# WU-CVGL/SIU3R

Hardware: AMD Instinct MI355X
Metric: image-pairs/sec @2x512^2 (SIU3R network forward incl. panoptic post-process) (higher is better)
Workload: dtype bf16x3 (fp32 activations, bf16 MFMA with hi/lo operand split; meets the 1e-3 parity bar)

## Files before the change

include/siu3r_hip.h:

```cpp
#ifndef SIU3R_HIP_H
#define SIU3R_HIP_H
#include <stdint.h>
#ifdef __cplusplus
extern "C" {
#endif

#define SIU3R_BF16 0
#define SIU3R_F32 1
#define SIU3R_F16 2
#define SIU3R_F64 3

const char* siu3r_last_error(void);
#define SIU3R_ABI_VERSION 12
int siu3r_abi_version(void);

int siu3r_rope2d(void* tokens, int dtype, int B, int N, int H, int D, int64_t stride_b,
                 int64_t stride_n, int64_t stride_h, const int64_t* positions, float base, float fwd,
                 void* stream);

typedef struct {
  const void* a;
  const void* w_hi;
  const void* w_lo;
  void* c;
// ... 62 lines not shown
int siu3r_layernorm2(const float* x, void* y, int y_dtype, void* y2_bf16, const float* gamma, const float* beta, int64_t rows, int C,
                     int64_t ldx, int64_t ldy, int64_t ldy2, float eps, void* stream);

typedef struct {
  const void *q, *k, *v;
  void* out;
  int32_t dtype;
  int32_t B, H, Nq, Nk, D;
  int64_t q_sb, q_sn, q_sh, k_sb, k_sn, k_sh, v_sb, v_sn, v_sh;
  float scale;
  const float *rope_cos, *rope_sin;
  int32_t rope_max_pos;
  const int64_t *qpos, *kpos;
  const uint8_t* mask;
  int32_t split3;
  int64_t mask_ld;
  float* ws;
  int32_t splits;
  int32_t kv_bxor;
  int32_t kv_x3;
  int32_t out_x3;
} siu3r_attn_params;
int siu3r_attention(const siu3r_attn_params* p, void* stream);
int siu3r_attention_out_x3_ok(const siu3r_attn_params* p);
int siu3r_attention_kv_x3_ok(const siu3r_attn_params* p);
typedef struct {
  char kernel[160];
  int32_t queries_per_wg, key_ranges, combine, key_halves, side_path;
} siu3r_attn_plan_t;
int siu3r_attention_plan(const siu3r_attn_params* p, siu3r_attn_plan_t* out);

int siu3r_add(const float* a, const float* b, float* y, int64_t rows, int64_t b_rows, int C, void* stream);
int siu3r_pack_image_nhwc(const float* img, void* out, int out_dtype, int N, int H, int W, int cpad, void* stream);
int siu3r_resize_bilinear(const void* x, int x_dtype, void* y, int y_dtype, const void* addend, int add_dtype,
                          const float* ch_scale, const float* ch_shift, int N, int IH, int IW, int OH, int OW,
                          int C, int align_corners, void* stream);
int siu3r_resize_bilinear_strided(const void* x, int x_dtype, void* y, int y_dtype, const void* addend, int add_dtype,
                                  const float* ch_scale, const float* ch_shift, int N, int IH, int IW, int OH, int OW,
                                  int C, int align_corners, int64_t x_batch_stride, int64_t addend_batch_stride, void* stream);
int siu3r_resize_bilinear_planes(const void* x, int x_dtype, void* y_planes, int N, int IH, int IW, int OH, int OW, int C, int align_corners,
                                 int64_t x_batch_stride, void* stream);
int siu3r_affine_add(const void* x, int x_dtype, const void* addend, int add_dtype, void* y, int y_dtype,
                     const float* ch_scale, const float* ch_shift, int64_t rows, int C, void* stream);
int siu3r_affine_add_strided(const void* x, int x_dtype, const void* addend, int add_dtype, void* y, int y_dtype,
                             const float* ch_scale, const float* ch_shift, int64_t rows, int C, int64_t rows_per_batch,
                             int64_t x_batch_stride, int64_t addend_batch_stride, void* stream);
int siu3r_maxpool3x3s2(const void* x, void* y, int dtype, int N, int IH, int IW, int C, void* stream);
int siu3r_maxpool2x2s2(const void* x, void* y, int dtype, int N, int IH, int IW, int C, void* stream);
int siu3r_lpips_layer(const float* f0, const float* f1, const float* w, float* dist, int64_t npix, int C, float eps, void* stream);
int siu3r_stem7x7_x3(const float* img, const void* wfrag, const float* bias, const float* up_src, float* out, int B, int G, int H, int W,
                     int planes_out, void* stream);
int siu3r_proj_rows_x3(const float* x, const void* wfrag, const float* bias, float* out, int Z, int G, int64_t M, int K, int N, int ldc,
                       int64_t out_z_stride, void* stream);
int siu3r_dwconv3x3_gelu(const void* x, void* y, int dtype, const float* w9c, const float* bias, int B, int H,
                         int W, int C, void* stream);
int siu3r_dwconv3x3_gelu_planes(const float* x, void* y_planes, const float* w9c, const float* bias, int B, int H, int W, int C, void* stream);
int siu3r_msdeform_sample(const void* value, int v_dtype, const float* offs_aw, const float* ref,
                          const int32_t* shapes_host, void* out, int out_dtype, int B, int S, int Q, int heads,
                          int d, int L, int P, void* stream);
int siu3r_msdeform_sample_planes(const void* value, int v_dtype, const float* offs_aw, const float* ref, const int32_t* shapes_host,
                                 void* out_planes, int B, int S, int Q, int heads, int d, int L, int P, void* stream);
int siu3r_groupnorm(const void* x, int x_dtype, void* y, int y_dtype, const float* gamma, const float* beta,
                    float* stats_ws, const void* addend, int add_dtype, int relu, int N, int HW, int C,
                    int groups, float eps, void* stream);
int siu3r_pts3d_exp(float* xyz, int64_t n, void* stream);
int siu3r_gaussian_adapter(const void* raw, int raw_dtype, float* opacities, float* scales, float* rotations,
                           float* harmonics, float* covariances, int64_t n, void* stream);
int siu3r_m2f_attn_mask(const float* mask_logits, uint8_t* out, int32_t* row_counts_ws, int B, int T, int IH,
                        int IW, int OH, int OW, int Q, int64_t out_ld, void* stream);

typedef struct {
  int32_t mode;
  int32_t width, height;
  float w2c[16];
  float proj[16];
  float tanfovx, tanfovy;
  float campos[3];
  float bg[3];
  int32_t sh_degree;
  int32_t sh_band4;
  float k2_znear_cull;
  float fx, fy, cx, cy;
  float near_plane, far_plane;
  float eps2d;
  float radius_clip;
  float extent_sigma;
  int32_t opacity_aware_extent;
  float alpha_min;
  float alpha_max;
  float t_min;
  float dilation;
  int32_t nt_post_blend;
  float k2_near, k2_far;
} siu3r_raster_cam;
int siu3r_raster_geometry(int width, int height, int64_t G, int32_t* out8);
int siu3r_raster_project(const siu3r_raster_cam* cams_host, int V, void* cams_dev, int64_t G, const float* means, const float* cov,
                         int cov_stride, const float* opacities, const float* colors, int channels, int sh_planar, float* rec,
                         int32_t* radii, int32_t* rect, int32_t* tiles_touched, uint32_t* keys, uint64_t* stats, void* stream);
int siu3r_raster_project_dp(const siu3r_raster_cam* cams_host, int V, void* cams_dev, const float* viewmats_dev, const float* Ks_dev, int64_t G,
                            const float* means, const float* cov, int cov_stride, const float* opacities, const float* colors, int channels,
                            int sh_planar, float* rec, int32_t* radii, int32_t* rect, int32_t* tiles_touched, uint32_t* keys, uint64_t* stats,
                            void* stream);
int siu3r_raster_project_c2w(const siu3r_raster_cam* cams_host, int V, void* cams_dev, const float* c2w_dev, const float* Kn_dev, float t_scale,
                             int64_t G, const float* means, const float* cov, int cov_stride, const float* opacities, const float* colors,
                             int channels, int sh_planar, float* rec, int32_t* radii, int32_t* rect, int32_t* tiles_touched, uint32_t* keys,
                             uint64_t* stats, void* stream);
// ... 158 lines not shown
```

siu3r_amd/_lib.py:

```python
from __future__ import annotations

import ctypes as C
import os

_HERE = os.path.dirname(os.path.abspath(__file__))
LIB_PATH = os.environ.get("SIU3R_LIB_OVERRIDE") or os.path.join(_HERE, "libsiu3r_hip.so")

BF16, F32 = 0, 1


class GemmParams(C.Structure):
    _fields_ = [
        ("a", C.c_void_p), ("w_hi", C.c_void_p), ("w_lo", C.c_void_p), ("c", C.c_void_p),
        ("bias", C.c_void_p), ("residual", C.c_void_p),
        ("m", C.c_int32), ("n", C.c_int32), ("k", C.c_int32), ("kpad", C.c_int32),
        ("lda", C.c_int64), ("ldc", C.c_int64), ("ldr", C.c_int64),
        ("a_dtype", C.c_int32), ("c_dtype", C.c_int32), ("r_dtype", C.c_int32),
        ("act", C.c_int32), ("relu_in", C.c_int32),
        ("batch", C.c_int32),
        ("sa", C.c_int64), ("sw", C.c_int64), ("sc", C.c_int64), ("sr", C.c_int64),
        ("a_mode", C.c_int32),
        ("ih", C.c_int32), ("iw", C.c_int32), ("cin", C.c_int32), ("kh", C.c_int32), ("kw", C.c_int32),
        ("stride", C.c_int32), ("pad", C.c_int32), ("oh", C.c_int32), ("ow", C.c_int32),
        ("out_mode", C.c_int32), ("up", C.c_int32), ("cout", C.c_int32),
# ... 41 lines not shown
        ("key_halves", C.c_int32), ("side_path", C.c_int32),
    ]


class RasterCam(C.Structure):
    _fields_ = [
        ("mode", C.c_int32), ("width", C.c_int32), ("height", C.c_int32),
        ("w2c", C.c_float * 16), ("proj", C.c_float * 16),
        ("tanfovx", C.c_float), ("tanfovy", C.c_float), ("campos", C.c_float * 3), ("bg", C.c_float * 3),
        ("sh_degree", C.c_int32), ("sh_band4", C.c_int32), ("k2_znear_cull", C.c_float),
        ("fx", C.c_float), ("fy", C.c_float), ("cx", C.c_float), ("cy", C.c_float),
        ("near_plane", C.c_float), ("far_plane", C.c_float), ("eps2d", C.c_float), ("radius_clip", C.c_float),
        ("extent_sigma", C.c_float), ("opacity_aware_extent", C.c_int32),
        ("alpha_min", C.c_float), ("alpha_max", C.c_float), ("t_min", C.c_float), ("dilation", C.c_float),
        ("nt_post_blend", C.c_int32), ("k2_near", C.c_float), ("k2_far", C.c_float),
    ]


class AdamField(C.Structure):
    _fields_ = [
        ("param", C.c_void_p), ("grad", C.c_void_p), ("exp_avg", C.c_void_p), ("exp_avg_sq", C.c_void_p),
        ("width", C.c_int32), ("head_period", C.c_int32), ("lr", C.c_float), ("lr_tail", C.c_float),
    ]


_P, _I, _L, _F = C.c_void_p, C.c_int, C.c_int64, C.c_float
ABI_VERSION = 12

SIGNATURES = {
    "siu3r_last_error": [],
    "siu3r_abi_version": [],
    "siu3r_rope2d": [_P, _I, _I, _I, _I, _I, _L, _L, _L, _P, _F, _F, _P],
    "siu3r_gemm": [C.POINTER(GemmParams), _P],
    "siu3r_gemm_plan": [C.POINTER(GemmParams), C.POINTER(GemmPlan)],
    "siu3r_gemm_tune": [_I, _I],
    "siu3r_layernorm": [_P, _P, _I, _P, _P, _L, _I, _L, _L, _F, _P],
    "siu3r_layernorm2": [_P, _P, _I, _P, _P, _P, _L, _I, _L, _L, _L, _F, _P],
    "siu3r_attention": [C.POINTER(AttnParams), _P],
    "siu3r_attention_kv_x3_ok": [C.POINTER(AttnParams)],
    "siu3r_attention_out_x3_ok": [C.POINTER(AttnParams)],
    "siu3r_attention_plan": [C.POINTER(AttnParams), C.POINTER(AttnPlan)],
    "siu3r_add": [_P, _P, _P, _L, _L, _I, _P],
    "siu3r_pack_image_nhwc": [_P, _P, _I, _I, _I, _I, _I, _P],
    "siu3r_resize_bilinear": [_P, _I, _P, _I, _P, _I, _P, _P, _I, _I, _I, _I, _I, _I, _I, _P],
    "siu3r_affine_add": [_P, _I, _P, _I, _P, _I, _P, _P, _L, _I, _P],
    "siu3r_resize_bilinear_strided": [_P, _I, _P, _I, _P, _I, _P, _P, _I, _I, _I, _I, _I, _I, _I, _L, _L, _P],
    "siu3r_resize_bilinear_planes": [_P, _I, _P, _I, _I, _I, _I, _I, _I, _I, _L, _P],
    "siu3r_affine_add_strided": [_P, _I, _P, _I, _P, _I, _P, _P, _L, _I, _L, _L, _L, _P],
    "siu3r_maxpool3x3s2": [_P, _P, _I, _I, _I, _I, _I, _P],
    "siu3r_maxpool2x2s2": [_P, _P, _I, _I, _I, _I, _I, _P],
    "siu3r_lpips_layer": [_P, _P, _P, _P, _L, _I, _F, _P],
    "siu3r_stem7x7_x3": [_P, _P, _P, _P, _P, _I, _I, _I, _I, _I, _P],
    "siu3r_proj_rows_x3": [_P, _P, _P, _P, _I, _I, _L, _I, _I, _I, _L, _P],
    "siu3r_dwconv3x3_gelu": [_P, _P, _I, _P, _P, _I, _I, _I, _I, _P],
    "siu3r_dwconv3x3_gelu_planes": [_P, _P, _P, _P, _I, _I, _I, _I, _P],
    "siu3r_msdeform_sample_planes": [_P, _I, _P, _P, C.POINTER(C.c_int32), _P, _I, _I, _I, _I, _I, _I, _I, _P],
    "siu3r_msdeform_sample": [_P, _I, _P, _P, C.POINTER(C.c_int32), _P, _I, _I, _I, _I, _I, _I, _I, _I, _P],
    "siu3r_groupnorm": [_P, _I, _P, _I, _P, _P, _P, _P, _I, _I, _I, _I, _I, _I, _F, _P],
    "siu3r_pts3d_exp": [_P, _L, _P],
    "siu3r_gaussian_adapter": [_P, _I, _P, _P, _P, _P, _P, _L, _P],
    "siu3r_m2f_attn_mask": [_P, _P, _P, _I, _I, _I, _I, _I, _I, _I, _L, _P],
    "siu3r_split_bf16": [_P, _P, _P, _P, _L, _I, _I, _L, _P],
    "siu3r_raster_geometry": [_I, _I, _L, C.POINTER(C.c_int32)],
    "siu3r_raster_project": [C.POINTER(RasterCam), _I, _P, _L, _P, _P, _I, _P, _P, _I, _I, _P, _P, _P, _P, _P, _P, _P],
    "siu3r_raster_sort": [_I, _L, _P, _P, _P, _P, _P, _P, _P, _P],
    "siu3r_raster_bin": [C.POINTER(RasterCam), _I, _L, _P, _P, _P, _P, _P, _P, _P, _L, _P, _P],
    "siu3r_raster_composite_rgb": [C.POINTER(RasterCam), _I, _P, _L, _P, _P, _L, _P, _P, _P, _P, _P, _P],
    "siu3r_raster_tile_lists": [C.POINTER(RasterCam), _I, _P, _P, _L, _P, _P, _P, _L, _P, _P],
    "siu3r_raster_composite_feat": [C.POINTER(RasterCam), _I, _P, _L, _P, _P, _L, _P, _P, _I, _P, _P, _P],
    "siu3r_raster_composite_feat_ws_bytes": [_I, _I, _I, _L],
    "siu3r_raster_tune": [_I, _I],
    "siu3r_raster_composite_feat_ws": [C.POINTER(RasterCam), _I, _P, _L, _P, _P, _L, _P, _P, _I, _P, _P, _P, _L, _P],
    "siu3r_scale_inplace": [_P, _L, _F, _P],
    "siu3r_quat_scale_to_cov6": [_P, _P, _P, _L, _P],
    "siu3r_sh_eval": [_P, _P, _P, _I, _I, _P, _L, _P],
    "siu3r_blend_background": [_P, _P, _P, _I, _L, _P],
    "siu3r_sh_eval_dp": [_P, _P, _P, _I, _I, _P, _L, _P],
    "siu3r_blend_background_dp": [_P, _P, _P, _I, _L, _P],
    "siu3r_raster_project_dp": [C.POINTER(RasterCam), _I, _P, _P, _P, _L, _P, _P, _I, _P, _P, _I, _I, _P, _P, _P, _P, _P, _P, _P],
    "siu3r_raster_project_c2w": [C.POINTER(RasterCam), _I, _P, _P, _P, _F, _L, _P, _P, _I, _P, _P, _I, _I, _P, _P, _P, _P, _P, _P, _P],
    "siu3r_raster_project_aa": [C.POINTER(RasterCam), _I, _P, _L, _P, _P, _I, _P, _P, _I, _I, _P, _P, _P, _P, _P, _P, _P, _P],
    "siu3r_raster_project_c2w_aa": [C.POINTER(RasterCam), _I, _P, _P, _P, _F, _L, _P, _P, _I, _P, _P, _I, _I, _P, _P, _P, _P, _P, _P, _P, _P],
    "siu3r_raster_project_bwd_aa": [C.POINTER(RasterCam), _I, _P, _L, _P, _P, _I, _P, _P, _I, _I, _P, _P, _P, _P, _P, _P, _P, _P, _P],
    "siu3r_mip_filter3d_ws": [_I],
    "siu3r_mip_filter3d": [_P, _P, _I, _I, _I, _P, _L, _F, _F, _F, _P, _P, _P],
    "siu3r_mip_apply": [_P, _P, _P, _L, _P, _P, _P],
    "siu3r_mip_apply_bwd": [_P, _P, _P, _P, _P, _L, _P, _P, _P],
    "siu3r_raster_composite_rgb_bwd": [C.POINTER(RasterCam), _I, _P, _L, _P, _P, _L, _P, _P, _P, _P, _P, _P, _P, _P, _P],
    "siu3r_raster_composite_rgb_bwd_abs": [C.POINTER(RasterCam), _I, _P, _L, _P, _P, _L, _P, _P, _P, _P, _P, _P, _P, _P, _P, _P],
    "siu3r_raster_contrib": [C.POINTER(RasterCam), _I, _P, _L, _P, _P, _L, _P, _P, _P, _P, _P],
    "siu3r_raster_project_bwd": [C.POINTER(RasterCam), _I, _P, _L, _P, _P, _I, _P, _P, _I, _I, _P, _P, _P, _P, _P, _P, _P, _P, _P],
    "siu3r_raster_pose_partial_rows": [_L],
    "siu3r_raster_pose_reduce": [_I, _L, _P, _P, _P],
    "siu3r_raster_composite_rgb_bwd_k3": [C.POINTER(RasterCam), _I, _P, _L, _P, _P, _L, _P, _P, _P, _P, _P, _P, _P],
    "siu3r_raster_composite_feat_ws_lists": [_I, _I, _I, _L, _P, _I, _P, _L, _L],
    "siu3r_raster_quad_lists": [C.POINTER(RasterCam), _I, _P, _L, _P, _P, _L, _P, _P, _L, _P],
    "siu3r_raster_composite_feat_bwd": [C.POINTER(RasterCam), _I, _P, _L, _P, _P, _L, _P, _P, _I, _P, _P, _P, _P, _P, _P, _P],
    "siu3r_raster_project_bwd_k3": [C.POINTER(RasterCam), _I, _P, _L, _P, _P, _I, _P, _P, _P, _P, _P, _P, _P, _P],
    "siu3r_raster_viewmat_reduce": [_I, _L, _P, _P, _P],
    "siu3r_quat_scale_to_cov6_bwd": [_P, _P, _P, _P, _P, _L, _P],
    "siu3r_sh_eval_bwd": [_P, _P, _P, _I, _I, _P, _P, _P, _P, _L, _P],
    "siu3r_photo_loss_partials": [_I, _I, _I, _I],
    "siu3r_photo_loss": [_P, _P, _I, _I, _I, _I, C.POINTER(C.c_int64), C.POINTER(C.c_int64), _F, _F, _P, _P, _P, _P],
    "siu3r_depth_loss_ws": [_I, _I, _I],
    "siu3r_depth_loss": [_P, _P, _P, _P, _I, _I, _I, _I, _I, _F, _P, _P, _P, _P, _P, _P, _P],
    "siu3r_depth_smooth_ws": [_I, _I, _I],
# ... 68 lines not shown
```

siu3r_amd/model.py:

```python
from __future__ import annotations

import functools
import math
from typing import Dict, List, Optional, Sequence

import os

import torch
import torch.nn.functional as F

from . import ops
from .ops import ACT_GELU, ACT_NONE, ACT_RELU
from .gaussians_types import Gaussians
from . import postprocess as pp

ENC_HEADS, DEC_HEADS = 16, 12
ADAPTER_IDX = (5, 11, 17, 23)
DPT_HOOKS = (0, 6, 9, 12)


class _Weights:

    def __init__(self, sd: Dict[str, torch.Tensor], device, split: bool):
        self.sd, self.dev, self.split = sd, device, split
# ... 5 lines not shown

    def v(self, name):
        if name not in self.vec:
            self.vec[name] = self.t(name).contiguous()
        return self.vec[name]

    def linear(self, name, key=None, extra_bias=None):
        key = key or name
        if key not in self.lin:
            w = self.t(name + ".weight")
            w = w.reshape(w.shape[0], -1)
            b = self.t(name + ".bias") if (name + ".bias") in self.sd else None
            if extra_bias is not None:
                b = extra_bias if b is None else b + extra_bias
            self.lin[key] = ops.pack_matrix(w, b, self.split)
        return self.lin[key]

    def linear_ln(self, names, ln_name, eps=1e-6):
        names = [names] if isinstance(names, str) else list(names)
        key = "+".join(names) + "#ln:" + ln_name
        if key not in self.lin:
            w = torch.cat([self.t(n + ".weight").reshape(self.sd[n + ".weight"].shape[0], -1) for n in names], 0)
            b = torch.cat([self.t(n + ".bias") for n in names], 0) if (names[0] + ".bias") in self.sd else None
            pw = ops.pack_linear_ln(w, b, self.t(ln_name + ".weight"), self.t(ln_name + ".bias"), self.split)
            pw.meta["ln_eps"] = eps
            self.lin[key] = pw
        return self.lin[key]

    def linear_ln_rows(self, name, rows, ln_name, eps=1e-6):
        key = f"{name}[{rows[0]}:{rows[1]}]#ln:{ln_name}"
        if key not in self.lin:
            w = self.t(name + ".weight")[rows[0]:rows[1]]
            b = self.t(name + ".bias")[rows[0]:rows[1]] if (name + ".bias") in self.sd else None
            pw = ops.pack_linear_ln(w, b, self.t(ln_name + ".weight"), self.t(ln_name + ".bias"), self.split)
            pw.meta["ln_eps"] = eps
            self.lin[key] = pw
        return self.lin[key]

    def group(self, key, build, prefixes):
        if key not in self.lin:
            self.lin[key] = ops.stack_packed([build(q) for q in prefixes])
        return self.lin[key]

    def stem7(self, names):
        key = "stem7:" + "|".join(names)
        if key not in self.lin:
            self.lin[key] = ops.pack_stem7([self.t(n + ".weight") for n in names], [self.t(n + ".bias") if (n + ".bias") in self.sd else None for n in names])
        return self.lin[key]

    def proj(self, names):
        key = "proj:" + "|".join(names)
        if key not in self.lin:
            self.lin[key] = ops.pack_proj([self.t(n + ".weight") for n in names], [self.t(n + ".bias") if (n + ".bias") in self.sd else None for n in names])
        return self.lin[key]

    def merged(self, key, names):
        if key not in self.lin:
            w = torch.cat([self.t(n + ".weight") for n in names], 0)
            b = torch.cat([self.t(n + ".bias") for n in names], 0)
            self.lin[key] = ops.pack_matrix(w, b, self.split)
        return self.lin[key]

    def conv(self, name, cin_pad=None, bn=None):
        if name not in self.lin:
            w = self.t(name + ".weight")
            b = self.t(name + ".bias") if (name + ".bias") in self.sd else None
            if bn is not None:
                s = self.t(bn + ".weight") / torch.sqrt(self.t(bn + ".running_var") + 1e-5)
                w = w * s[:, None, None, None]
                b0 = b if b is not None else torch.zeros_like(s)
                b = (b0 - self.t(bn + ".running_mean")) * s + self.t(bn + ".bias")
            self.lin[name] = ops.pack_conv(w, b, self.split, cin_pad=cin_pad)
        return self.lin[name]

    def convT(self, name):
        if name not in self.lin:
            self.lin[name] = ops.pack_conv_transpose(self.t(name + ".weight"), self.t(name + ".bias"), self.split)
        return self.lin[name]

    def bn_affine(self, name):
        key = name + "#affine"
        if key not in self.vec:
            s = self.t(name + ".weight") / torch.sqrt(self.t(name + ".running_var") + 1e-5)
            self.vec[key] = s.contiguous()
            self.vec[key + "b"] = (self.t(name + ".bias") - self.t(name + ".running_mean") * s).contiguous()
        return self.vec[key], self.vec[key + "b"]


class _Ctx:
    def __init__(self, w: _Weights, precision: str):
        assert precision in ("bf16", "bf16x3")
        self.w = w
        self.precision = precision
        self.split = precision == "bf16x3"
        self.act = torch.float32 if self.split else torch.bfloat16
        self.dev = w.dev
        self.cache: Dict = {}
        self._streams: Dict = {}
        self.concurrent = os.environ.get("SIU3R_NO_STREAMS", "0") != "1"
        self.fold = os.environ.get("SIU3R_NO_LNFOLD", "0") != "1"

    def side_stream(self, i):
        k = i
        if k not in self._streams:
            self._streams[k] = torch.cuda.Stream(device=self.dev)
        return self._streams[k]
# ... 614 lines not shown
        f1 = None
        if with_f1:
            s1, b1 = ctx.w.bn_affine("adapter.norm1")
            c1 = ops.linear(a["c1_feat"], ctx.w.linear("adapter.spm.fc1"), out_dtype=torch.float32)
            c1 = ops.conv_transpose2d(c2, ctx.w.convT("adapter.up"), out_dtype=torch.float32, residual=c1)
            f1 = ops.resize_bilinear(x1, (4 * h, 4 * w), False, addend=c1, ch_scale=s1, ch_shift=b1, out_dtype=ctx.act)
        f2 = ops.resize_bilinear(x2, (2 * h, 2 * w), False, addend=c2, ch_scale=s2, ch_shift=b2, out_dtype=ctx.act)
        f3 = ops.affine_add(x3, c3, s3, b3, out_dtype=ctx.act)
        f4 = ops.resize_bilinear(x4, (h // 2, w // 2), False, addend=c4, ch_scale=s4, ch_shift=b4, out_dtype=ctx.act)
        return [f1, f2, f3, f4]

    def forward_nhwc(self, img: torch.Tensor, img8: torch.Tensor, all_feat: Sequence[torch.Tensor]):
        a = self.spm(img8)
        for i, idx in enumerate(ADAPTER_IDX):
            self.interact(a, i, all_feat[idx])
        return self.finish(a, with_f1=True)

    def forward(self, x, all_feat):
        img8 = ops.pack_image_nhwc(x.contiguous().float(), self.ctx.act, ops.image_channels(self.ctx.split))
        return [f.permute(0, 3, 1, 2) for f in self.forward_nhwc(x, img8, all_feat)]

    __call__ = forward


def _sine_pos_2d(h, w, npf=128):
    y = torch.arange(1, h + 1, dtype=torch.float32)[:, None].expand(h, w)
    x = torch.arange(1, w + 1, dtype=torch.float32)[None, :].expand(h, w)
    eps, scale = 1e-6, 2 * math.pi
    y = y / (y[-1:, :] + eps) * scale
    x = x / (x[:, -1:] + eps) * scale
    dim_t = torch.arange(npf, dtype=torch.float32)
    dim_t = 10000 ** (2 * torch.div(dim_t, 2, rounding_mode="floor") / npf)
    px, py = x[:, :, None] / dim_t, y[:, :, None] / dim_t
    px = torch.stack((px[:, :, 0::2].sin(), px[:, :, 1::2].cos()), dim=3).flatten(2)
    py = torch.stack((py[:, :, 0::2].sin(), py[:, :, 1::2].cos()), dim=3).flatten(2)
    return torch.cat((py, px), dim=2).reshape(h * w, 2 * npf)


def _sine_pos_3d(t, h, w, npf=128):
    z = torch.arange(1, t + 1, dtype=torch.float32)[:, None, None].expand(t, h, w)
    y = torch.arange(1, h + 1, dtype=torch.float32)[None, :, None].expand(t, h, w)
    x = torch.arange(1, w + 1, dtype=torch.float32)[None, None, :].expand(t, h, w)
    eps, scale = 1e-6, 2 * math.pi
    y = y / (y[:, -1:, :] + eps) * scale
    x = x / (x[:, :, -1:] + eps) * scale
    z = z / (z[-1:, :, :] + eps) * scale
    dim_t = torch.arange(npf, dtype=torch.float32)
    dim_t = 10000 ** (2 * torch.div(dim_t, 2, rounding_mode="floor") / npf)
    dim_tz = torch.arange(npf * 2, dtype=torch.float32)
    dim_tz = 10000 ** (2 * torch.div(dim_tz, 2, rounding_mode="floor") / (npf * 2))
    px, py, pz = x[..., None] / dim_t, y[..., None] / dim_t, z[..., None] / dim_tz
    f = lambda p_: torch.stack((p_[..., 0::2].sin(), p_[..., 1::2].cos()), dim=4).flatten(3)
    return (torch.cat((f(py), f(px)), dim=3) + f(pz)).reshape(t * h * w, 2 * npf)


class VideoMask2FormerForVideoSegmentationOutput(dict):

    __getattr__ = dict.get


class VideoMask2FormerForVideoSegmentation:
    def __init__(self, ctx: _Ctx, num_queries=100):
        self.ctx, self.num_queries = ctx, num_queries
        self.forced_attn_masks = None
        self.record_attn_masks = None
        self.heads = 8

    def _pixel_decoder(self, feats, lat1=None):
        ctx = self.ctx
        pd = "mask2former.model.pixel_decoder"
        N2 = feats[1].shape[0]
        lv = list(feats)[::-1][:3]
        shapes = [(f.shape[1], f.shape[2]) for f in lv]
        S = sum(a * b for a, b in shapes)
        key = ("pd_const", tuple(shapes))
        if key not in ctx.cache:
            le = ctx.w.t(pd + ".level_embed").cpu()
            pos = torch.cat([_sine_pos_2d(a, b) + le[i] for i, (a, b) in enumerate(shapes)], 0)
            pts = []
            for (hh, ww) in shapes:
                ry, rx = torch.meshgrid(torch.linspace(0.5, hh - 0.5, hh), torch.linspace(0.5, ww - 0.5, ww), indexing="ij")
                pts.append(torch.stack((rx.reshape(-1) / ww, ry.reshape(-1) / hh), -1))
            ref = torch.cat(pts, 0)[:, None, :].expand(-1, 3, -1).contiguous()
            ctx.cache[key] = (pos.contiguous().to(ctx.dev), ref.to(ctx.dev))
        pos, ref = ctx.cache[key]
        hs = torch.empty((N2, S, 256), dtype=torch.float32, device=ctx.dev)
        o = 0
        for lvl, x in enumerate(lv):
            e = ops.linear(x, ctx.w.linear(f"{pd}.input_projections.{lvl}.0"), out_dtype=torch.float32)
            e = ops.groupnorm(e, ctx.w.v(f"{pd}.input_projections.{lvl}.1.weight"), ctx.w.v(f"{pd}.input_projections.{lvl}.1.bias"))
            n = shapes[lvl][0] * shapes[lvl][1]
            hs[:, o:o + n] = e.view(N2, n, 256)
            o += n
        hsb = hs if ctx.split else hs.to(ctx.act)
        for i in range(6):
            p = f"{pd}.encoder.layers.{i}"
            wkey = p + ".self_attn.offs_aw0"
            if wkey not in ctx.w.lin:
                w_oa = torch.cat((ctx.w.t(p + ".self_attn.sampling_offsets.weight"), ctx.w.t(p + ".self_attn.attention_weights.weight")), 0)
                b_oa = torch.cat((ctx.w.t(p + ".self_attn.sampling_offsets.bias"), ctx.w.t(p + ".self_attn.attention_weights.bias")), 0)
                ctx.w.lin[wkey] = ops.pack_matrix(w_oa, None, ctx.split)
                ctx.cache[wkey] = (w_oa, b_oa)
            rkey = (wkey, tuple(shapes))
            if rkey not in ctx.cache:
                w_oa, b_oa = ctx.cache[wkey]
                ctx.cache[rkey] = (pos @ w_oa.t() + b_oa).contiguous()
            pres = ctx.cache[rkey]
            offs_aw = ops.linear(hsb, ctx.w.lin[wkey], out_dtype=torch.float32, residual=pres if N2 == 1 else pres[None].expand(N2, -1, -1))
            value = ops.linear(hsb, ctx.w.linear(p + ".self_attn.value_proj"), out_dtype=ctx.act)
            samp = ops.msdeform_sample(value, offs_aw, ref, shapes, 8, 4, ctx.act)
            a = ops.linear(samp, ctx.w.linear(p + ".self_attn.output_proj"), out_dtype=torch.float32, residual=hs)
            hs, hsb = ctx.ln2(p + ".self_attn_layer_norm", a, 1e-5)
            f_ = ops.linear(hsb, ctx.w.linear(p + ".fc1"), out_dtype=ctx.act, act=ACT_RELU)
            f_ = ops.linear(f_, ctx.w.linear(p + ".fc2"), out_dtype=torch.float32, residual=hs)
            hs, hsb = ctx.ln2(p + ".final_layer_norm", f_, 1e-5)
        outs, o = [], 0
        for (hh, ww) in shapes:
            outs.append(hs[:, o:o + hh * ww].contiguous().view(N2, hh, ww, 256))
            o += hh * ww
        lat = lat1 if lat1 is not None else ops.linear(feats[0], ctx.w.linear(pd + ".adapter_1.0"), out_dtype=torch.float32)
        up = ops.resize_bilinear(outs[-1], (lat.shape[1], lat.shape[2]), False)
        out = ops.groupnorm(lat, ctx.w.v(pd + ".adapter_1.1.weight"), ctx.w.v(pd + ".adapter_1.1.bias"), addend=up, out_dtype=ctx.act)
        out = ops.conv2d(out, ctx.w.conv(pd + ".layer_1.0"), pad=1, out_dtype=torch.float32)
        out = ops.groupnorm(out, ctx.w.v(pd + ".layer_1.1.weight"), ctx.w.v(pd + ".layer_1.1.bias"), relu=True, out_dtype=ctx.act)
        mask_features = ops.linear(out, ctx.w.linear(pd + ".mask_projection"), out_dtype=torch.float32)
        return mask_features, outs

    def _mask_predictor(self, inter, mask_features_bt, size):
        ctx = self.ctx
        p = "mask2former.model.transformer_module.decoder.mask_predictor.mask_embedder"
        e = ops.linear(inter, ctx.w.linear(p + ".0.0"), out_dtype=ctx.act, act=ACT_RELU)
        e = ops.linear(e, ctx.w.linear(p + ".1.0"), out_dtype=ctx.act, act=ACT_RELU)
        if ctx.split:
            e = ops.linear(e, ctx.w.linear(p + ".2.0"), out_dtype=torch.float32)
            B, Q, Cc = e.shape
            hi, lo, kpad, x3 = ops.split_bf16(e.view(B * Q, Cc), True, want_x3=True)
        else:
            hi, lo, x3 = ops.linear(e, ctx.w.linear(p + ".2.0"), out_dtype=torch.bfloat16), None, None
            B, Q, Cc = hi.shape
            kpad = Cc
        m = ops.bmm_nt(mask_features_bt, hi.view(B, Q, kpad), None if lo is None else lo.view(B, Q, kpad), Q, Cc, b_x3=x3)
        m = m.view(B, self._T, self._H4, self._W4, Q)
        am = ops.m2f_attn_mask(m, size) if size is not None else None
        return m, am

    def _decoder(self, ms, mask_features, B, T):
        ctx = self.ctx
        tm = "mask2former.model.transformer_module"
        dp = tm + ".decoder"
        H4, W4 = mask_features.shape[1], mask_features.shape[2]
        self._T, self._H4, self._W4 = T, H4, W4
        mf_bt = mask_features.view(B, T * H4 * W4, 256)
        if not ctx.split:
            mf_bt = mf_bt.to(ctx.act)
        sizes = [(f.shape[1], f.shape[2]) for f in ms]
        key = ("m2f_pos3d", T, tuple(sizes))
        if key not in ctx.cache:
            ctx.cache[key] = [_sine_pos_3d(T, a, b).contiguous().to(ctx.dev) for (a, b) in sizes]
        pos3 = ctx.cache[key]
        le = ctx.w.v(tm + ".level_embed.weight")
        if "ones256" not in ctx.cache:
            ctx.cache["ones256"] = torch.ones(256, device=ctx.dev)
        ones = ctx.cache["ones256"]
# ... 458 lines not shown
```

siu3r_amd/ops.py:

```python
from __future__ import annotations

import ctypes as C
import math
import os
from dataclasses import dataclass
from typing import Optional, Sequence

import torch

from . import _lib
from ._lib import BF16, F32, AttnParams, GemmParams, check

ACT_NONE, ACT_GELU, ACT_RELU = 0, 1, 2


def _dt(t: torch.Tensor) -> int:
    if t.dtype == torch.float32:
        return F32
    if t.dtype == torch.bfloat16:
        return BF16
    raise RuntimeError(f"unsupported dtype {t.dtype} (float32 or bfloat16 expected)")


def torch_dtype(code: int):
# ... 668 lines not shown

def add(a: torch.Tensor, b: torch.Tensor):
    _gpu(a, b)
    assert a.is_contiguous() and b.is_contiguous() and a.dtype == torch.float32 and b.dtype == torch.float32
    Cc = a.shape[-1]
    y = torch.empty_like(a)
    check(_lib.lib().siu3r_add(_p(a), _p(b), _p(y), a.numel() // Cc, b.numel() // Cc, Cc, _stream()))
    return y


def pack_image_nhwc(img: torch.Tensor, out_dtype, cpad: int = 8):
    _gpu(img)
    assert img.dtype == torch.float32 and img.is_contiguous() and img.shape[1] == 3
    N, _, H, W = img.shape
    out = torch.empty((N, H, W, cpad), dtype=out_dtype, device=img.device)
    check(_lib.lib().siu3r_pack_image_nhwc(_p(img), _p(out), _dt(out), N, H, W, cpad, _stream()))
    return out


def pack_image_nhwc8(img: torch.Tensor, out_dtype):
    return pack_image_nhwc(img, out_dtype, 8)


def pack_stem7(weights: Sequence[torch.Tensor], biases: Sequence[Optional[torch.Tensor]]):
    frs = []
    for w in weights:
        _gpu(w)
        assert tuple(w.shape) == (256, 3, 7, 7), w.shape
        wk = torch.zeros((256, 7, 8, 4), dtype=torch.float32, device=w.device)
        wk[:, :, :7, :3] = w.detach().float().permute(0, 2, 3, 1)
        wk = wk.reshape(256, 14, 2, 8)
        fr = wk.reshape(8, 32, 14, 2, 8).permute(0, 2, 3, 1, 4)
        fr = fr.reshape(8, 14, 64, 8)
        hi = fr.to(torch.bfloat16)
        lo = (fr - hi.float()).to(torch.bfloat16)
        frs.append(torch.stack([hi, lo], dim=2))
    b = None
    if any(x is not None for x in biases):
        b = torch.stack([torch.zeros(256, device=weights[0].device) if x is None else x.detach().float() for x in biases]).contiguous()
    return torch.stack(frs).contiguous(), b


def stem7x7_x3(img: torch.Tensor, wfrag: torch.Tensor, bias: Optional[torch.Tensor], up_src: Optional[torch.Tensor], out: torch.Tensor, planes: bool = False):
    _gpu(img, wfrag, bias, up_src, out)
    B, G, H, W, c = img.shape
    assert c == 4 and img.dtype == torch.float32 and img.is_contiguous() and tuple(wfrag.shape) == (G, 8, 14, 2, 64, 8) and wfrag.dtype == torch.bfloat16
    assert out.shape == (B, G, H, W, 256) and out.dtype == torch.float32 and out.is_contiguous()
    assert bias is None or (tuple(bias.shape) == (G, 256) and bias.is_contiguous())
    assert up_src is None or (up_src.shape == (B, G, H // 2, W // 2, 256) and up_src.dtype == torch.float32 and up_src.is_contiguous())
    check(_lib.lib().siu3r_stem7x7_x3(_p(img), _p(wfrag), _p(bias), _p(up_src), _p(out), B, G, H, W, 1 if planes else 0, _stream()))
    return out


def pack_proj(weights: Sequence[torch.Tensor], biases: Sequence[Optional[torch.Tensor]]):
    frs, N = [], None
    for w in weights:
        _gpu(w)
        w = w.detach().float().reshape(w.shape[0], -1)
        N, K = w.shape
        NB = (N + 31) // 32
        assert K % 16 == 0
        wp = torch.zeros((NB * 32, K), dtype=torch.float32, device=w.device)
        wp[:N] = w
        fr = wp.reshape(NB, 32, K // 16, 2, 8).permute(0, 2, 3, 1, 4).reshape(NB, K // 16, 64, 8)
        hi = fr.to(torch.bfloat16)
        lo = (fr - hi.float()).to(torch.bfloat16)
        frs.append(torch.stack([hi, lo], dim=2))
    b = None
    if any(x is not None for x in biases):
        NB = frs[0].shape[0]
        b = torch.zeros((len(weights), NB * 32), dtype=torch.float32, device=frs[0].device)
        for i, x in enumerate(biases):
            if x is not None:
                b[i, :N] = x.detach().float()
    return torch.stack(frs).contiguous(), b, N


def proj_rows_x3(x: torch.Tensor, wfrag: torch.Tensor, bias: Optional[torch.Tensor], n: int, out: torch.Tensor):
    _gpu(x, wfrag, bias, out)
    B, G, M, K = x.shape
    assert x.dtype == torch.float32 and x.is_contiguous() and wfrag.shape[0] == G and wfrag.dtype == torch.bfloat16
    assert out.shape == (B, G, M, n) and out.dtype == torch.float32 and out.stride(3) == 1 and out.stride(2) >= n
    zs = out.stride(1) if G > 1 else out.stride(0)
    assert zs >= M * out.stride(2) and (B == 1 or G == 1 or out.stride(0) == G * zs), (out.shape, out.stride())
    check(_lib.lib().siu3r_proj_rows_x3(_p(x), _p(wfrag), _p(bias), _p(out), B * G, G, M, K, n, out.stride(2), zs, _stream()))
    return out


def proj_rows_ok(K: int, n: int) -> bool:
    return (K == 256 and 65 <= n <= 96) or (K == 128 and n <= 32)


def image_channels(split: bool) -> int:
    return 4 if split else 8


def _batch_strided(t: torch.Tensor, inner: int) -> int:
    dense = list(torch.empty(t.shape[1:], device="meta").stride())
    assert list(t.stride()[1:]) == dense and (t.shape[0] == 1 or t.stride(0) >= inner), (t.shape, t.stride())
    return t.stride(0) if t.shape[0] > 1 else inner


def resize_bilinear(x: torch.Tensor, size, align_corners: bool, *, addend=None, ch_scale=None, ch_shift=None,
                    out_dtype=None, out: Optional[torch.Tensor] = None, planes_out: Optional[Planes] = None, planes_only: bool = False):
    _gpu(x, addend, out)
    N, IH, IW, Cc = x.shape
    OH, OW = size
    if out is None:
        out = torch.empty((N, OH, OW, Cc), dtype=out_dtype or x.dtype, device=x.device)
    assert out.shape == (N, OH, OW, Cc) and out.is_contiguous()
    x_bs = _batch_strided(x, IH * IW * Cc)
    if _producer_planes(planes_out, planes_only, out, lambda: addend is None and ch_scale is None and Cc % 32 == 0 and planes_out.t.data_ptr() % 128 == 0):
        check(_lib.lib().siu3r_resize_bilinear_planes(_p(x), _dt(x), _p(planes_out.t), N, IH, IW, OH, OW, Cc, int(align_corners), x_bs, _stream()))
        return out
    a_bs = OH * OW * Cc
    if addend is not None:
        assert addend.shape == out.shape
        a_bs = _batch_strided(addend, OH * OW * Cc)
    check(_lib.lib().siu3r_resize_bilinear_strided(_p(x), _dt(x), _p(out), _dt(out), _p(addend), _dt(addend) if addend is not None else F32,
                                                   _p(ch_scale), _p(ch_shift), N, IH, IW, OH, OW, Cc, int(align_corners), x_bs, a_bs, _stream()))
    return out


def affine_add(x: torch.Tensor, addend, ch_scale, ch_shift, out_dtype=None):
    _gpu(x, addend)
    Cc = x.shape[-1]
    rows_pb = math.prod(x.shape[1:-1])
    x_bs = _batch_strided(x, rows_pb * Cc)
    a_bs = rows_pb * Cc
    if addend is not None:
        assert addend.numel() == x.numel()
        a_bs = _batch_strided(addend.view(x.shape) if addend.is_contiguous() else addend, rows_pb * Cc)
    out = torch.empty(x.shape, dtype=out_dtype or x.dtype, device=x.device)
    check(_lib.lib().siu3r_affine_add_strided(_p(x), _dt(x), _p(addend), _dt(addend) if addend is not None else F32, _p(out), _dt(out), _p(ch_scale),
                                              _p(ch_shift), x.shape[0] * rows_pb, Cc, rows_pb, x_bs, a_bs, _stream()))
    return out


def maxpool3x3s2(x: torch.Tensor):
    _gpu(x)
    assert x.is_contiguous()
    N, IH, IW, Cc = x.shape
    out = torch.empty((N, (IH - 1) // 2 + 1, (IW - 1) // 2 + 1, Cc), dtype=x.dtype, device=x.device)
# ... 131 lines not shown
```

Before: 55.16.

## Fuse deformable-attention output proj, layernorm and FFN into one rowchain kernel

Adds a HIP kernel that, for a 64-row tile, runs the output projection plus residual, layernorm, fc1 with ReLU, fc2 plus residual and the final layernorm in a single launch. The hidden FFN activations stay in LDS in 256-wide chunks and are never written to global memory. Weights are prepacked as bf16 hi/lo fragments, and the MFMA loop prefetches the next weight group. This removes several launches and the global round trips between them in the Mask2Former pixel decoder encoder layers. The cost is a large LDS footprint per block, and the path is used only in split mode with contiguous fp32 inputs.

```diff
diff --git a/include/siu3r_hip.h b/include/siu3r_hip.h
--- a/include/siu3r_hip.h
+++ b/include/siu3r_hip.h
@@ -138,6 +138,7 @@
                      int planes_out, void* stream);
 int siu3r_proj_rows_x3(const float* x, const void* wfrag, const float* bias, float* out, int Z, int G, int64_t M, int K, int N, int ldc,
                        int64_t out_z_stride, void* stream);
+int siu3r_rowchain_x3(const float* x, const float* res, const void* pack, float* out, int64_t M, int H, float eps1, float eps2, void* stream);
 int siu3r_dwconv3x3_gelu(const void* x, void* y, int dtype, const float* w9c, const float* bias, int B, int H,
                          int W, int C, void* stream);
 int siu3r_dwconv3x3_gelu_planes(const float* x, void* y_planes, const float* w9c, const float* bias, int B, int H, int W, int C, void* stream);
diff --git a/siu3r_amd/_lib.py b/siu3r_amd/_lib.py
--- a/siu3r_amd/_lib.py
+++ b/siu3r_amd/_lib.py
@@ -117,6 +117,7 @@
     "siu3r_lpips_layer": [_P, _P, _P, _P, _L, _I, _F, _P],
     "siu3r_stem7x7_x3": [_P, _P, _P, _P, _P, _I, _I, _I, _I, _I, _P],
     "siu3r_proj_rows_x3": [_P, _P, _P, _P, _I, _I, _L, _I, _I, _I, _L, _P],
+    "siu3r_rowchain_x3": [_P, _P, _P, _P, _L, _I, _F, _F, _P],
     "siu3r_dwconv3x3_gelu": [_P, _P, _I, _P, _P, _I, _I, _I, _I, _P],
     "siu3r_dwconv3x3_gelu_planes": [_P, _P, _P, _P, _I, _I, _I, _I, _P],
     "siu3r_msdeform_sample_planes": [_P, _I, _P, _P, C.POINTER(C.c_int32), _P, _I, _I, _I, _I, _I, _I, _I, _P],
diff --git a/siu3r_amd/csrc/rowchain.hip b/siu3r_amd/csrc/rowchain.hip
--- /dev/null
+++ b/siu3r_amd/csrc/rowchain.hip
@@ -0,0 +1,226 @@
+#include "common.h"
+
+namespace {
+
+constexpr int RC_D = 256;
+constexpr int RC_ROWS = 64;
+constexpr int RC_LD = RC_D + 8;
+constexpr int RC_PLANE = RC_ROWS * RC_LD + 32;
+constexpr int RC_LDF = RC_D + 4;
+static_assert(2 * RC_PLANE * 2 >= RC_ROWS * RC_LDF * 4, "the fp32 staging overlays the hidden chunk's planes");
+
+struct RowchainParams {
+  const float *x, *res;
+  const uint4 *wo, *w1, *w2;
+  const float *bo, *g1, *b1, *c2, *g2, *b2, *c1;
+  float* out;
+  int64_t M;
+  int H;
+  float eps1, eps2;
+};
+
+__device__ __forceinline__ void rc_barrier() { asm volatile("s_waitcnt lgkmcnt(0)\n\ts_barrier" ::: "memory"); }
+
+__device__ __forceinline__ float rc_wave_sum(float v) {
+#pragma unroll
+  for (int o = 32; o > 0; o >>= 1) v += __shfl_xor(v, o);
+  return v;
+}
+
+__device__ __forceinline__ void rc_load_w(uint4 (&wb)[8], const uint4* src) {
+#pragma unroll
+  for (int j = 0; j < 8; ++j) wb[j] = src[(j >> 1) * 128 + (j & 1) * 64];
+}
+
+__device__ __forceinline__ void rc_pass(const u16* a_hi, const u16* a_lo, const uint4* w, const uint4* w_next, uint4 (&wb)[8], f32x16 (&acc)[2]) {
+  uint4 a[4], an[4];
+  auto load_a = [&](uint4 (&d)[4], int ks) {
+    d[0] = *(const uint4*)(a_hi + 16 * ks);
+    d[1] = *(const uint4*)(a_lo + 16 * ks);
+    d[2] = *(const uint4*)(a_hi + 32 * RC_LD + 16 * ks);
+    d[3] = *(const uint4*)(a_lo + 32 * RC_LD + 16 * ks);
+  };
+  load_a(a, 0);
+#pragma unroll
+  for (int g = 0; g < 4; ++g) {
+    uint4 wn[8];
+    rc_load_w(wn, g < 3 ? w + (g + 1) * 4 * 128 : w_next);
+#pragma unroll
+    for (int s = 0; s < 4; ++s) {
+      const int ks = 4 * g + s;
+      if (ks < 15) load_a(an, ks + 1);
+      const bf16x8 bh = as_bf16x8(wb[2 * s]), bl = as_bf16x8(wb[2 * s + 1]);
+      acc[0] = __builtin_amdgcn_mfma_f32_32x32x16_bf16(as_bf16x8(a[0]), bh, acc[0], 0, 0, 0);
+      acc[1] = __builtin_amdgcn_mfma_f32_32x32x16_bf16(as_bf16x8(a[2]), bh, acc[1], 0, 0, 0);
+      acc[0] = __builtin_amdgcn_mfma_f32_32x32x16_bf16(as_bf16x8(a[0]), bl, acc[0], 0, 0, 0);
+      acc[1] = __builtin_amdgcn_mfma_f32_32x32x16_bf16(as_bf16x8(a[2]), bl, acc[1], 0, 0, 0);
+      acc[0] = __builtin_amdgcn_mfma_f32_32x32x16_bf16(as_bf16x8(a[1]), bh, acc[0], 0, 0, 0);
+      acc[1] = __builtin_amdgcn_mfma_f32_32x32x16_bf16(as_bf16x8(a[3]), bh, acc[1], 0, 0, 0);
+      if (ks < 15) {
+#pragma unroll
+        for (int i = 0; i < 4; ++i) a[i] = an[i];
+      }
+    }
+#pragma unroll
+    for (int j = 0; j < 8; ++j) wb[j] = wn[j];
+  }
+}
+
+template <bool FINAL>
+__device__ __forceinline__ void rc_layernorm(float* f, u16* s_hi, u16* s_lo, const float* gamma, const float* beta, float eps, float* out,
+                                             int64_t row0, int64_t M, int wave, int lane) {
+  const float4 g = *(const float4*)(gamma + 4 * lane), bb = *(const float4*)(beta + 4 * lane);
+#pragma unroll
+  for (int rr = 0; rr < 8; ++rr) {
+    const int r = 8 * wave + rr;
+    float* fr = f + r * RC_LDF + 4 * lane;
+    const float4 v = *(const float4*)fr;
+    float sum = 0.f;
+    sum += v.x + v.y + v.z + v.w;
+    const float mean = rc_wave_sum(sum) / (float)RC_D;
+    const float a = v.x - mean, b = v.y - mean, cc = v.z - mean, d = v.w - mean;
+    float sq = 0.f;
+    sq += a * a + b * b + cc * cc + d * d;
+    const float rstd = rsqrtf(rc_wave_sum(sq) / (float)RC_D + eps);
+    const float4 o = make_float4((v.x - mean) * rstd * g.x + bb.x, (v.y - mean) * rstd * g.y + bb.y, (v.z - mean) * rstd * g.z + bb.z,
+                                 (v.w - mean) * rstd * g.w + bb.w);
+    if (FINAL) {
+      if (row0 + r < M) *(float4*)(out + (row0 + r) * RC_D + 4 * lane) = o;
+    } else {
+      *(float4*)fr = o;
+      uint2 h, l;
+      split_trunc_bf16x2(o.x, o.y, h.x, l.x);
+      split_trunc_bf16x2(o.z, o.w, h.y, l.y);
+      *(uint2*)(s_hi + r * RC_LD + 4 * lane) = h;
+      *(uint2*)(s_lo + r * RC_LD + 4 * lane) = l;
+    }
+  }
+}
+
+__global__ __launch_bounds__(512) void rowchain_x3_kernel(const RowchainParams p) {
+#if __HIP_DEVICE_COMPILE__
+  __shared__ __attribute__((aligned(16))) u16 s_a[2 * RC_PLANE], s_h[2 * RC_PLANE];
+  float* s_f = (float*)s_h;
+  const int t = threadIdx.x, lane = t & 63, wave = t >> 6;
+  const int l31 = lane & 31, lh = lane >> 5;
+  const int col = 32 * wave + l31;
+  const int64_t row0 = (int64_t)blockIdx.x * RC_ROWS;
+  const int chunks = p.H / RC_D, ks2 = p.H / 16;
+
+  const uint4* w_cur = p.wo + (size_t)(wave * 16) * 128 + lane;
+  uint4 wb[8];
+  rc_load_w(wb, w_cur);
+  f32x16 rz[2];
+#pragma unroll
+  for (int b = 0; b < 2; ++b)
+#pragma unroll
+    for (int r = 0; r < 16; ++r) {
+      const int64_t row = row0 + 32 * b + (r & 3) + 8 * (r >> 2) + 4 * lh;
+      rz[b][r] = row < p.M ? p.res[row * RC_D + col] : 0.f;
+    }
+  {
+    constexpr int PPT = RC_ROWS * RC_D / 4 / 512;
+    float4 nx[PPT];
+#pragma unroll
+    for (int i = 0; i < PPT; ++i) {
+      const int pc = i * 512 + t;
+      const int64_t row = row0 + pc / (RC_D / 4);
+      nx[i] = row < p.M ? *(const float4*)(p.x + row * RC_D + 4 * (pc % (RC_D / 4))) : make_float4(0.f, 0.f, 0.f, 0.f);
+    }
+#pragma unroll
+    for (int i = 0; i < PPT; ++i) {
+      const int pc = i * 512 + t, r = pc / (RC_D / 4), c = 4 * (pc % (RC_D / 4));
+      uint2 h, l;
+      split_trunc_bf16x2(nx[i].x, nx[i].y, h.x, l.x);
+      split_trunc_bf16x2(nx[i].z, nx[i].w, h.y, l.y);
+      *(uint2*)(s_a + r * RC_LD + c) = h;
+      *(uint2*)(s_a + RC_PLANE + r * RC_LD + c) = l;
+    }
+  }
+  rc_barrier();
+
+  const int frag = l31 * RC_LD + 8 * lh;
+  const u16 *aa_hi = s_a + frag, *aa_lo = s_a + RC_PLANE + frag, *ah_hi = s_h + frag, *ah_lo = s_h + RC_PLANE + frag;
+  const uint4* w1_0 = p.w1 + (size_t)(wave * 16) * 128 + lane;
+  const uint4* w2_0 = p.w2 + (size_t)(wave * ks2) * 128 + lane;
+  f32x16 acc[2], acc2[2];
+  auto zero = [](f32x16 (&v)[2]) {
+#pragma unroll
+    for (int b = 0; b < 2; ++b)
+#pragma unroll
+      for (int r = 0; r < 16; ++r) v[b][r] = 0.f;
+  };
+  auto frow = [&](int b, int r) { return 32 * b + (r & 3) + 8 * (r >> 2) + 4 * lh; };
+
+  zero(acc);
+  rc_pass(aa_hi, aa_lo, w_cur, w1_0, wb, acc);
+  {
+    const float bv = p.bo[col];
+#pragma unroll
+    for (int b = 0; b < 2; ++b)
+#pragma unroll
+      for (int r = 0; r < 16; ++r) s_f[frow(b, r) * RC_LDF + col] = acc[b][r] + bv + rz[b][r];
+  }
+  rc_barrier();
+  rc_layernorm<false>(s_f, s_a, s_a + RC_PLANE, p.g1, p.b1, p.eps1, nullptr, row0, p.M, wave, lane);
+  rc_barrier();
+#pragma unroll
+  for (int b = 0; b < 2; ++b)
+#pragma unroll
+    for (int r = 0; r < 16; ++r) rz[b][r] = s_f[frow(b, r) * RC_LDF + col];
+
+  zero(acc2);
+  const bool odd = (lane & 1) != 0;
+  u16* hdst = s_h + (odd ? RC_PLANE : 0) + 32 * wave + (l31 & ~1);
+  for (int c = 0; c < chunks; ++c) {
+    const uint4* w1c = w1_0 + (size_t)c * (8 * 16 * 128);
+    const uint4* w2c = w2_0 + (size_t)c * (16 * 128);
+    zero(acc);
+    rc_pass(aa_hi, aa_lo, w1c, w2c, wb, acc);
+    const float cv = p.c1[c * RC_D + col];
+    rc_barrier();
+#pragma unroll
+    for (int b = 0; b < 2; ++b)
+#pragma unroll
+      for (int r = 0; r < 16; ++r) {
+        const float v = fmaxf(acc[b][r] + cv, 0.f);
+        const float nb = __int_as_float(__builtin_amdgcn_update_dpp(0, __float_as_int(v), 0xB1 , 0xF, 0xF, true));
+        uint32_t hi, lo;
+        split_trunc_bf16x2(odd ? nb : v, odd ? v : nb, hi, lo);
+        *(uint32_t*)(hdst + frow(b, r) * RC_LD) = odd ? lo : hi;
+      }
+    rc_barrier();
+    rc_pass(ah_hi, ah_lo, w2c, c + 1 < chunks ? w1c + 8 * 16 * 128 : w2c, wb, acc2);
+  }
+
+  rc_barrier();
+  {
+    const float bv = p.c2[col];
+#pragma unroll
+    for (int b = 0; b < 2; ++b)
+#pragma unroll
+      for (int r = 0; r < 16; ++r) s_f[frow(b, r) * RC_LDF + col] = acc2[b][r] + bv + rz[b][r];
+  }
+  rc_barrier();
+  rc_layernorm<true>(s_f, nullptr, nullptr, p.g2, p.b2, p.eps2, p.out, row0, p.M, wave, lane);
+#endif
+}
+
+}
+
+extern "C" int siu3r_rowchain_x3(const float* x, const float* res, const void* pack, float* out, int64_t M, int H, float eps1, float eps2,
+                                 void* stream) {
+  SIU3R_CHECK(M > 0 && cdiv64(M, RC_ROWS) <= 0x7fffffff, "rowchain_x3: bad row count M=%lld", (long long)M);
+  SIU3R_CHECK(H > 0 && H % RC_D == 0, "rowchain_x3: H=%d must be a positive multiple of 256", H);
+  SIU3R_CHECK(x && res && pack && out, "rowchain_x3: null pointer");
+  auto al16 = [](const void* q) { return ((uintptr_t)q & 15) == 0; };
+  SIU3R_CHECK(al16(x) && al16(res) && al16(pack) && al16(out), "rowchain_x3: x, res, pack and out must be 16-byte aligned");
+  const char* pk = (const char*)pack;
+  const size_t wo_b = (size_t)RC_D * RC_D * 4, w1_b = (size_t)H * RC_D * 4;
+  const float* vec = (const float*)(pk + wo_b + 2 * w1_b);
+  RowchainParams p{x, res, (const uint4*)pk, (const uint4*)(pk + wo_b), (const uint4*)(pk + wo_b + w1_b),
+                   vec, vec + RC_D, vec + 2 * RC_D, vec + 3 * RC_D, vec + 4 * RC_D, vec + 5 * RC_D, vec + 6 * RC_D, out, M, H, eps1, eps2};
+  hipLaunchKernelGGL(rowchain_x3_kernel, dim3((unsigned)cdiv64(M, RC_ROWS)), dim3(512), 0, (hipStream_t)stream, p);
+  SIU3R_LAUNCH_CHECK("siu3r_rowchain_x3");
+  return 0;
+}
diff --git a/siu3r_amd/model.py b/siu3r_amd/model.py
--- a/siu3r_amd/model.py
+++ b/siu3r_amd/model.py
@@ -81,6 +81,17 @@
         key = "proj:" + "|".join(names)
         if key not in self.lin:
             self.lin[key] = ops.pack_proj([self.t(n + ".weight") for n in names], [self.t(n + ".bias") if (n + ".bias") in self.sd else None for n in names])
+        return self.lin[key]
+
+    def rowchain(self, p):
+        key = "rowchain:" + p
+        if key not in self.lin:
+            t = self.t
+            self.lin[key] = (ops.pack_rowchain(t(p + ".self_attn.output_proj.weight"), t(p + ".self_attn.output_proj.bias"),
+                                               t(p + ".self_attn_layer_norm.weight"), t(p + ".self_attn_layer_norm.bias"),
+                                               t(p + ".fc1.weight"), t(p + ".fc1.bias"), t(p + ".fc2.weight"), t(p + ".fc2.bias"),
+                                               t(p + ".final_layer_norm.weight"), t(p + ".final_layer_norm.bias")),
+                             self.sd[p + ".fc1.weight"].shape[0])
         return self.lin[key]
 
     def merged(self, key, names):
@@ -801,6 +812,9 @@
     px, py, pz = x[..., None] / dim_t, y[..., None] / dim_t, z[..., None] / dim_tz
     f = lambda p_: torch.stack((p_[..., 0::2].sin(), p_[..., 1::2].cos()), dim=4).flatten(3)
     return (torch.cat((f(py), f(px)), dim=3) + f(pz)).reshape(t * h * w, 2 * npf)
+
+
+_ROWCHAIN = os.environ.get("SIU3R_NO_ROWCHAIN", "0") != "1"
 
 
 class VideoMask2FormerForVideoSegmentationOutput(dict):
@@ -858,6 +872,10 @@
             offs_aw = ops.linear(hsb, ctx.w.lin[wkey], out_dtype=torch.float32, residual=pres if N2 == 1 else pres[None].expand(N2, -1, -1))
             value = ops.linear(hsb, ctx.w.linear(p + ".self_attn.value_proj"), out_dtype=ctx.act)
             samp = ops.msdeform_sample(value, offs_aw, ref, shapes, 8, 4, ctx.act)
+            if _ROWCHAIN and ops.rowchain_ok(samp, hs, ctx.split):
+                pack, H = ctx.w.rowchain(p)
+                hs = hsb = ops.rowchain_x3(samp, hs, pack, H, 1e-5, 1e-5)
+                continue
             a = ops.linear(samp, ctx.w.linear(p + ".self_attn.output_proj"), out_dtype=torch.float32, residual=hs)
             hs, hsb = ctx.ln2(p + ".self_attn_layer_norm", a, 1e-5)
             f_ = ops.linear(hsb, ctx.w.linear(p + ".fc1"), out_dtype=ctx.act, act=ACT_RELU)
diff --git a/siu3r_amd/ops.py b/siu3r_amd/ops.py
--- a/siu3r_amd/ops.py
+++ b/siu3r_amd/ops.py
@@ -744,20 +744,25 @@
     return out
 
 
+def _proj_fragments(w: torch.Tensor) -> torch.Tensor:
+    w = w.detach().float().reshape(w.shape[0], -1)
+    N, K = w.shape
+    NB = (N + 31) // 32
+    assert K % 16 == 0
+    wp = torch.zeros((NB * 32, K), dtype=torch.float32, device=w.device)
+    wp[:N] = w
+    fr = wp.reshape(NB, 32, K // 16, 2, 8).permute(0, 2, 3, 1, 4).reshape(NB, K // 16, 64, 8)
+    hi = fr.to(torch.bfloat16)
+    lo = (fr - hi.float()).to(torch.bfloat16)
+    return torch.stack([hi, lo], dim=2)
+
+
 def pack_proj(weights: Sequence[torch.Tensor], biases: Sequence[Optional[torch.Tensor]]):
     frs, N = [], None
     for w in weights:
         _gpu(w)
-        w = w.detach().float().reshape(w.shape[0], -1)
-        N, K = w.shape
-        NB = (N + 31) // 32
-        assert K % 16 == 0
-        wp = torch.zeros((NB * 32, K), dtype=torch.float32, device=w.device)
-        wp[:N] = w
-        fr = wp.reshape(NB, 32, K // 16, 2, 8).permute(0, 2, 3, 1, 4).reshape(NB, K // 16, 64, 8)
-        hi = fr.to(torch.bfloat16)
-        lo = (fr - hi.float()).to(torch.bfloat16)
-        frs.append(torch.stack([hi, lo], dim=2))
+        N = w.shape[0]
+        frs.append(_proj_fragments(w))
     b = None
     if any(x is not None for x in biases):
         NB = frs[0].shape[0]
@@ -781,6 +786,49 @@
 
 def proj_rows_ok(K: int, n: int) -> bool:
     return (K == 256 and 65 <= n <= 96) or (K == 128 and n <= 32)
+
+
+def pack_rowchain(wo, bo, g1, b1, w1, c1, w2, c2, g2, b2) -> torch.Tensor:
+    H = w1.shape[0]
+    assert tuple(wo.shape) == (256, 256) and tuple(w1.shape) == (H, 256) and tuple(w2.shape) == (256, H) and H > 0 and H % 256 == 0
+    vec = [bo, g1, b1, c2, g2, b2, c1]
+    assert all(v.numel() == (H if v is c1 else 256) for v in vec)
+    parts = [_proj_fragments(w).contiguous().view(torch.uint8).reshape(-1) for w in (wo, w1, w2)]
+    parts.append(torch.cat([v.detach().float().reshape(-1) for v in vec]).contiguous().view(torch.uint8))
+    return torch.cat(parts).contiguous()
+
+
+def unpack_rowchain(pack: torch.Tensor, H: int) -> dict:
+    def mat(buf, N, K):
+        fr = buf.view(torch.bfloat16).reshape(N // 32, K // 16, 2, 2, 32, 8).double()
+        return (fr[:, :, 0] + fr[:, :, 1]).permute(0, 3, 1, 2, 4).reshape(N, K)
+    pack = pack.cpu()
+    o1, o2, o3 = 256 * 256 * 4, 256 * 256 * 4 + H * 256 * 4, 256 * 256 * 4 + 2 * H * 256 * 4
+    assert pack.dtype == torch.uint8 and pack.numel() == o3 + (6 * 256 + H) * 4
+    vec = pack[o3:].view(torch.float32)
+    out = {"wo": mat(pack[:o1], 256, 256), "w1": mat(pack[o1:o2], H, 256), "w2": mat(pack[o2:o3], 256, H)}
+    for i, k in enumerate(("bo", "g1", "b1", "c2", "g2", "b2")):
+        out[k] = vec[256 * i:256 * (i + 1)].clone()
+    out["c1"] = vec[6 * 256:].clone()
+    return out
+
+
+def rowchain_ok(x: torch.Tensor, res: torch.Tensor, split: bool) -> bool:
+    return bool(split) and all(t.dtype == torch.float32 and t.is_contiguous() and t.dim() >= 2 and t.shape[-1] == 256 for t in (x, res)) \
+        and x.shape == res.shape
+
+
+def rowchain_x3(x: torch.Tensor, res: torch.Tensor, pack: torch.Tensor, H: int, eps1: float, eps2: float, out: Optional[torch.Tensor] = None):
+    _gpu(x, res, pack, out)
+    assert rowchain_ok(x, res, True), (x.shape, x.dtype, res.shape, res.dtype)
+    assert pack.dtype == torch.uint8 and pack.numel() == (256 * 256 + 2 * H * 256) * 4 + (6 * 256 + H) * 4
+    if out is None:
+        out = torch.empty_like(x)
+    assert out.shape == x.shape and out.dtype == torch.float32 and out.is_contiguous()
+    M = x.numel() // 256
+    if M:
+        check(_lib.lib().siu3r_rowchain_x3(_p(x), _p(res), _p(pack), _p(out), M, H, eps1, eps2, _stream()))
+    return out
 
 
 def image_channels(split: bool) -> int:
```

New measurement: 55.93 (median of 6 runs). +1.4%, better.
